# tue-mps/simple-tad

Hardware: AMD Instinct MI355X
Metric: clips/sec (16x224^2 ViT-B) fwd+bwd (higher is better)
Workload: dtype bf16; 1 GPU; vit_base_patch16_224 16x224x224, 32 clips/GPU, fwd+bwd+AdamW fine-tune step with CE loss on synthetic labels (BASELINE configs[2]/[3]); global_batch=32, per_gpu_batch=32, parallelism=dp1, residual_stream=f32, operands=bf16, parameters=86228738

## Files before the change

simple_tad_amd/_lib.py:

```python
from __future__ import annotations

import ctypes as C
import os

_HERE = os.path.dirname(os.path.abspath(__file__))
LIB_PATH = os.environ.get("TAD_LIB") or os.path.join(_HERE, "libtad_mi355x.so")

_vp, _i, _i64, _f, _sz = C.c_void_p, C.c_int, C.c_int64, C.c_float, C.c_size_t

SIGNATURES = {
    "tad_abi_version": (_i, []),
    "tad_last_error_string": (C.c_char_p, []),
    "tad_cast_f32_bf16": (_i, [_vp, _vp, _i64, _vp]),
    "tad_transpose_cast_f32_bf16": (_i, [_vp, _vp, _i, _i, _vp]),
    "tad_patch_embed_ldk": (_i, [_i, _i, _i]),
    "tad_im2col_tubelets": (_i, [_vp, _vp, _i, _i, _i, _i, _i, _i, _i, _vp]),
    "tad_im2col_tubelets_16": (_i, [_vp, _vp, _i, _i, _i, _i, _i, _i, _i, _vp]),
    "tad_patch_embed_fwd": (_i, [_vp, _vp, _vp, _vp, _vp, _vp, _i, _i, _i, _i, _i, _i, _i, _i, _vp]),
    "tad_patch_embed_fwd_implicit": (_i, [_vp, _vp, _vp, _vp, _vp, _i, _i, _i, _i, _i, _i, _i, _i, _vp]),
    "tad_im2col_tubelets_u8": (_i, [_vp, _vp, _i, _i, _i, _i, _i, _i, C.POINTER(_f), C.POINTER(_f), _i, _i, _vp]),
    "tad_im2col_frame_windows": (_i, [_vp, _i64, _vp, _vp, _i, _i, _i, _i, _i, _i, _i, C.POINTER(_f), C.POINTER(_f), _i, _vp]),
    "tad_patch_embed_gemm": (_i, [_vp, _vp, _vp, _vp, _vp, _i64, _i, _i, _i, _vp]),
    "tad_patch_embed_bwd_workspace_bytes": (_sz, [_i64, _i, _i]),
    "tad_patch_embed_bwd": (_i, [_vp, _vp, _vp, _vp, _vp, _sz, _i64, _i, _i, _vp]),
# ... 111 lines not shown
for _bf, _h in (*F16_TWINS.items(), *VARIANT_F16_TWINS.items()):
    SIGNATURES[_h] = SIGNATURES[_bf]
EPI_BIAS, EPI_BIAS_GELU, EPI_BIAS_RESIDUAL = 0, 1, 2
ABI_VERSION = 5

EXT_SIGNATURES = {
    "tadx_abi_version": (_i, []),
    "tadx_rmsnorm_fwd": (_i, [_vp, _vp, _vp, _i, _vp, _i64, _i, _f, _vp]),
    "tadx_rmsnorm_bwd_workspace_bytes": (_sz, [_i64, _i]),
    "tadx_rmsnorm_bwd": (_i, [_vp, _i, _vp, _vp, _vp, _vp, _vp, _vp, _i, _vp, _i, _vp, _sz, _i64, _i, _vp]),
    "tadx_qk_rmsnorm_fwd": (_i, [_vp, _vp, _vp, _vp, _i, _vp, _f, _i64, _i, _f, _vp]),
    "tadx_qk_rmsnorm_bwd_workspace_bytes": (_sz, [_i64, _i]),
    "tadx_qk_rmsnorm_bwd": (_i, [_vp, _i, _vp, _vp, _vp, _vp, _f, _vp, _vp, _vp, _i, _vp, _sz, _i64, _i, _vp]),
}
EXT_ABI_VERSION = 1
LINEAR_PLAN_FIELDS = ("r0", "rows", "kernel", "persistent", "direct", "grid", "block", "group_m", "sk_splits", "sk_mode", "epilogue")
ATTN_PLAN_FIELDS = ("kernel", "hd", "out16", "qs", "drop", "dma_mode", "skip", "has_lo", "grid", "block")
ATTN_FWD, ATTN_FWD_Q64, ATTN_BWD_DQ, ATTN_BWD_DKV = range(4)
LINEAR_BWD_WEIGHT_PLAN_FIELDS = ("N", "tile_k", "tiles", "tiles_k", "splits", "rows_per_split", "kernel", "grid", "block", "pair", "ws_lo", "ws_hi")
ADAMW_CHUNK = 4096
ADAMW_MAX_GROUPS = 128
EMA_CHUNK = 8192
MIXUP_PLAN_WORDS = 12
MIX_KEEP, MIX_BLEND, MIX_PASTE = 0, 1, 2
FRAME_LOSS_KINDS = {"focal": 0, "focal2": 1, "exponential": 2, "2bce": 3, "smoothap": 4}
ERASE_BOX_WORDS = 8
ERASE_CONST, ERASE_RAND, ERASE_PIXEL = 0, 1, 2
RANDAUG_ROW_WORDS = 20
RANDAUG_MAX_LAYERS = 32
(RA_COPY, RA_INVERT, RA_POSTERIZE, RA_SOLARIZE, RA_SOLARIZE_ADD, RA_AUTOCONTRAST, RA_EQUALIZE, RA_BRIGHTNESS, RA_COLOR, RA_CONTRAST,
# ... 12 lines not shown


class TadError(RuntimeError):
    pass


def load() -> C.CDLL:
    global _lib
    if _lib is not None:
        return _lib
    if not os.path.exists(LIB_PATH):
        raise TadError(
            f"{LIB_PATH} not found: the HIP extension has not been built. Run `python -m simple_tad_amd.build` "
            "(or __graft_entry__.build()). There is no CPU fallback for the MI355X path.")
    lib = C.CDLL(LIB_PATH)
    for name, (res, args) in (*SIGNATURES.items(), *EXT_SIGNATURES.items()):
        try:
            fn = getattr(lib, name)
        except AttributeError as e:
            raise TadError(f"{LIB_PATH} does not export {name}") from e
        fn.restype = res
        fn.argtypes = args
    v = lib.tad_abi_version()
    if v != ABI_VERSION:
        raise TadError(f"ABI mismatch: library reports {v}, binding expects {ABI_VERSION}")
    v = lib.tadx_abi_version()
    if v != EXT_ABI_VERSION:
        raise TadError(f"extension ABI mismatch: library reports {v}, binding expects {EXT_ABI_VERSION}")
    _lib = lib
    return lib


def check(rc: int, what: str = "") -> None:
    if rc != 0:
        msg = load().tad_last_error_string()
        raise TadError(f"{what} failed (rc={rc}): {msg.decode() if msg else ''}")
```

simple_tad_amd/build.py:

```python
import os
import subprocess
import sys
from concurrent.futures import ThreadPoolExecutor

HERE = os.path.dirname(os.path.abspath(__file__))
CSRC = os.path.join(HERE, "csrc")
_ABLATION = os.environ.get("TAD_BUILD_ABLATION") == "1"
_LIB_NAME = os.environ.get("TAD_BUILD_LIB", "libtad_ablation.so" if _ABLATION else "libtad_mi355x.so")
EXP_DIR = os.path.join(os.path.dirname(HERE), "build_exp")
_PRODUCTION = _LIB_NAME == "libtad_mi355x.so"
LIB = os.path.join(HERE if _PRODUCTION else EXP_DIR, os.path.basename(_LIB_NAME))
SOURCES = ["capi.hip", "elementwise.hip", "patch_embed.hip", "layernorm.hip", "gemm.hip", "gemm_plan.hip", "gemm_w4.hip", "attn_fwd.hip", "attn_bwd.hip", "attn_plan.hip", "attn_f32.hip", "precise.hip", "optim.hip", "ema.hip", "mixup.hip", "frame_loss.hip", "erasing.hip", "randaug.hip", "multiscale_crop.hip", "frame_resize.hip", "spatial_sample.hip", "mae.hip", "metrics.hip", "group_metrics.hip", "grad_segnorm.hip", "collective.hip", "im2col.hip", "pooled_tail.hip", "layerscale.hip", "attn_colsum.hip", "rmsnorm.hip"]
F16_SOURCES = ["elementwise.hip", "patch_embed.hip", "layernorm.hip", "gemm.hip", "gemm_w4.hip", "attn_fwd.hip", "attn_bwd.hip", "optim.hip", "pooled_tail.hip", "layerscale.hip"]
NO_VGPR_FORM = {"gemm_w4.hip"}
EXTRA_DEPS = {"gemm.hip": ["gemm_kernels.h", "gemm_plan.h"], "gemm_w4.hip": ["gemm_kernels.h", "gemm_plan.h"], "gemm_plan.hip": ["gemm_plan.h", "knob.h"],
              "attn_fwd.hip": ["attn_plan.h"], "attn_bwd.hip": ["attn_plan.h"], "attn_plan.hip": ["attn_plan.h", "knob.h"],
              "multiscale_crop.hip": ["frame_io.h"], "frame_resize.hip": ["frame_io.h"], "spatial_sample.hip": ["frame_io.h"], "randaug.hip": ["frame_io.h"],
              "rmsnorm.hip": ["../../include/tad_mi355x_ext.h"]}
NO_FP_CONTRACT = {"ema.hip", "mixup.hip", "randaug.hip", "multiscale_crop.hip", "spatial_sample.hip", "frame_resize.hip"}
FLAGS = ["--offload-arch=gfx950", "-O3", "-std=c++17", "-fPIC", "-ffp-contract=fast", "-Wno-unused-result",
         "-mllvm", "-amdgpu-mfma-vgpr-form=1"]


def _hipcc():
    for c in (os.environ.get("HIPCC"), "/opt/rocm/bin/hipcc", "hipcc"):
        if c and (os.path.isabs(c) and os.path.exists(c) or not os.path.isabs(c)):
            return c
    return "hipcc"


def _deps_mtime():
    m = 0.0
    for root in (CSRC, os.path.join(os.path.dirname(HERE), "include")):
# ... 46 lines not shown
```

simple_tad_amd/csrc/layernorm.hip:

```cpp
#include "common.h"

TAD_NAMESPACE_BEGIN

constexpr int LN_MAX_V = 8;

int launch_reduce_partials(const float* partial, float* out, int splits, int64_t n, int accumulate, hipStream_t st);
int launch_reduce_cols(const float* partial, float* out0, float* out1, float* out2, int nq, int splits, int n, int accumulate,
                       hipStream_t st);

template <int NV, bool OUT_BF16>
__global__ __launch_bounds__(256) void layernorm_fwd_kernel(const float* __restrict__ x, const float* __restrict__ gamma,
                                                            const float* __restrict__ beta, void* __restrict__ y,
                                                            float* __restrict__ mean, float* __restrict__ rstd,
                                                            int64_t rows, int D, float eps) {
  const int lane = threadIdx.x & 63;
  const int64_t row = (int64_t)blockIdx.x * 4 + (threadIdx.x >> 6);
  if (row >= rows) return;
  const int D4 = D >> 2;
  const float4* xr = reinterpret_cast<const float4*>(x + row * D);
  float4 v[NV];
  float s = 0.f;
#pragma unroll
  for (int i = 0; i < NV; ++i) {
    const int c = lane + 64 * i;
// ... 27 lines not shown
      o.z = (v[i].z - mu) * rs * g.z + b.z;
      o.w = (v[i].w - mu) * rs * g.w + b.w;
      if (OUT_BF16) {
        uint2 p;
        p.x = pack_op16x2(o.x, o.y);
        p.y = pack_op16x2(o.z, o.w);
        stg_u2<false>(reinterpret_cast<uint2*>((uint16_t*)y + row * D) + c, p);
      } else {
        stg_f4<false>(reinterpret_cast<float4*>((float*)y + row * D) + c, o);
      }
    }
  }
}

__device__ const float ln_one = 1.0f;
template <int NV, bool DY_BF16, bool FULL>
__global__ __launch_bounds__(256) void layernorm_bwd_kernel(const void* __restrict__ dy, const float* __restrict__ x,
                                                            const float* __restrict__ gamma, const float* __restrict__ mean,
                                                            const float* __restrict__ rstd, const float* __restrict__ dres,
                                                            float* __restrict__ dx, uint16_t* __restrict__ dxb,
                                                            float* __restrict__ partial , int64_t rows, int D,
                                                            int rows_per_block, int want_colsum,
                                                            const float* __restrict__ rowscale, int rows_per_scale) {
  extern __shared__ __attribute__((aligned(16))) float smem[];
  const int lane = threadIdx.x & 63, wave = __builtin_amdgcn_readfirstlane(threadIdx.x >> 6);
  const int D4 = D >> 2;
  const int64_t r0 = (int64_t)blockIdx.x * rows_per_block;
  const int64_t r1 = min(rows, r0 + rows_per_block);
  float4 g[NV], dg[NV], db[NV], cs[NV];
#pragma unroll
  for (int i = 0; i < NV; ++i) {
    const int c = lane + 64 * i;
    g[i] = (c < D4) ? reinterpret_cast<const float4*>(gamma)[c] : make_float4(0.f, 0.f, 0.f, 0.f);
    dg[i] = db[i] = cs[i] = make_float4(0.f, 0.f, 0.f, 0.f);
  }
  const float* const rsrc = dres ? dres : x;
  const float rmul = dres ? 1.f : 0.f;
  const float* const scp = rowscale ? rowscale : &ln_one;
  int sidx = 0, srem = 0;
  if (rowscale) {
    sidx = (int)((r0 + wave) / rows_per_scale);
    srem = (int)((r0 + wave) - (int64_t)sidx * rows_per_scale);
  }
  for (int64_t row = r0 + wave; row < r1; row += 4) {
    float4 xv[NV], dyv[NV], rv[NV];
    uint2 dyp[NV];
#pragma unroll
    for (int i = 0; i < NV; ++i) {
      const int c = lane + 64 * i;
      if (FULL || c < D4) {
        xv[i] = ldg_f4<false>(reinterpret_cast<const float4*>(x + row * D) + c);
        if (DY_BF16) dyp[i] = ldg_u2<false>(reinterpret_cast<const uint2*>((const uint16_t*)dy + row * D) + c);
        else dyv[i] = ldg_f4<false>(reinterpret_cast<const float4*>((const float*)dy + row * D) + c);
        rv[i] = ldg_f4<false>(reinterpret_cast<const float4*>(rsrc + row * D) + c);
      }
    }
    const float mu = mean[row], rs = rstd[row];
    const float sc = scp[sidx];
    if (rowscale) {
      srem += 4;
      while (srem >= rows_per_scale) { srem -= rows_per_scale; ++sidx; }
    }
    __builtin_amdgcn_sched_barrier(0);
    float4 xh[NV];
    float s1 = 0.f, s2 = 0.f;
#pragma unroll
    for (int i = 0; i < NV; ++i) {
      const int c = lane + 64 * i;
      if (FULL || c < D4) {
        if (DY_BF16)
          dyv[i] = make_float4(op16_lo_f32(dyp[i].x), op16_hi_f32(dyp[i].x), op16_lo_f32(dyp[i].y), op16_hi_f32(dyp[i].y));
        xh[i] = make_float4((xv[i].x - mu) * rs, (xv[i].y - mu) * rs, (xv[i].z - mu) * rs, (xv[i].w - mu) * rs);
        const float4 t = make_float4(dyv[i].x * g[i].x, dyv[i].y * g[i].y, dyv[i].z * g[i].z, dyv[i].w * g[i].w);
        s1 += (t.x + t.y) + (t.z + t.w);
        s2 += (t.x * xh[i].x + t.y * xh[i].y) + (t.z * xh[i].z + t.w * xh[i].w);
        dg[i].x += dyv[i].x * xh[i].x; dg[i].y += dyv[i].y * xh[i].y; dg[i].z += dyv[i].z * xh[i].z; dg[i].w += dyv[i].w * xh[i].w;
// ... 51 lines not shown
    for (int w = 1; w < 4; ++w) {
      const float4 b = sm[(w * 3 + q) * D4 + c];
      a.x += b.x; a.y += b.y; a.z += b.z; a.w += b.w;
    }
    reinterpret_cast<float4*>(partial + ((int64_t)q * gridDim.x + blockIdx.x) * D)[c] = a;
  }
}

static inline int ln_bwd_blocks(int64_t rows) {
  int64_t b = (rows + 31) / 32;
  if (b > 1024) b = 1024;
  if (b < 1) b = 1;
  return (int)b;
}

TAD_NAMESPACE_END

using namespace tad;

extern "C" {

int tad_layernorm_fwd(const float* x, const float* gamma, const float* beta, void* y, int y_dtype, float* mean, float* rstd,
                      int64_t rows, int D, float eps, tad_stream_t stream) {
  TAD_REQUIRE(x && gamma && beta && y, "layernorm_fwd: null pointer");
  TAD_REQUIRE(rows > 0 && D > 0 && D % 4 == 0 && D <= 64 * 4 * LN_MAX_V, "layernorm_fwd: D=%d must be a multiple of 4 and <= %d", D,
              64 * 4 * LN_MAX_V);
  TAD_REQUIRE(y_dtype == TAD_F32 || y_dtype == TAD_OP16, "layernorm_fwd: bad y_dtype %d", y_dtype);
  TAD_REQUIRE_ALIGNED("layernorm_fwd", x, 16);
  TAD_REQUIRE_ALIGNED("layernorm_fwd", gamma, 16);
  TAD_REQUIRE_ALIGNED("layernorm_fwd", beta, 16);
  TAD_REQUIRE_ALIGNED("layernorm_fwd", y, y_dtype == TAD_F32 ? 16 : 8);
// ... 14 lines not shown
    case 6: LN_FWD(6); break;
    default: LN_FWD(8); break;
  }
#undef LN_FWD
  return check_launch("layernorm_fwd");
}

#ifndef TAD_OPND_F16
size_t tad_layernorm_bwd_workspace_bytes(int64_t rows, int D) { return (size_t)3 * ln_bwd_blocks(rows) * (size_t)D * sizeof(float); }
#endif

int tad_layernorm_bwd(const void* dy, int dy_dtype, const float* x, const float* gamma, const float* mean, const float* rstd,
                      const float* dres, float* dx, uint16_t* dx_bf16, float* dgamma, float* dbeta, float* colsum_dx,
                      const float* rowscale, int rows_per_scale, int accumulate, void* ws, size_t ws_bytes, int64_t rows, int D,
                      tad_stream_t stream) {
  TAD_REQUIRE(dy && x && gamma && mean && rstd && dx && dgamma && dbeta && ws, "layernorm_bwd: null pointer");
  TAD_REQUIRE(rows > 0 && D > 0 && D % 4 == 0 && D <= 64 * 4 * LN_MAX_V, "layernorm_bwd: unsupported D=%d", D);
  TAD_REQUIRE(dy_dtype == TAD_F32 || dy_dtype == TAD_OP16, "layernorm_bwd: bad dy_dtype %d", dy_dtype);
  TAD_REQUIRE(!rowscale || rows_per_scale > 0, "layernorm_bwd: rows_per_scale must be positive");
  TAD_REQUIRE_ALIGNED("layernorm_bwd", dy, dy_dtype == TAD_F32 ? 16 : 8);
  TAD_REQUIRE_ALIGNED("layernorm_bwd", x, 16);
  TAD_REQUIRE_ALIGNED("layernorm_bwd", gamma, 16);
  TAD_REQUIRE_ALIGNED("layernorm_bwd", dres, 16);
  TAD_REQUIRE_ALIGNED("layernorm_bwd", dx, 16);
  TAD_REQUIRE_ALIGNED("layernorm_bwd", dx_bf16, 8);
  TAD_REQUIRE_ALIGNED("layernorm_bwd", dgamma, 16);
  TAD_REQUIRE_ALIGNED("layernorm_bwd", dbeta, 16);
  TAD_REQUIRE_ALIGNED("layernorm_bwd", colsum_dx, 16);
  TAD_REQUIRE_ALIGNED("layernorm_bwd", ws, 16);
  const int blocks = ln_bwd_blocks(rows);
  if (ws_bytes < (size_t)3 * blocks * D * sizeof(float)) { set_error("layernorm_bwd: workspace too small"); return TAD_ENOSPACE; }
  const int rows_per_block = (int)((rows + blocks - 1) / blocks);
  const int nv = (D / 4 + 63) / 64;
  const size_t smem = (size_t)4 * 3 * D * sizeof(float);
  hipStream_t st = (hipStream_t)stream;
  float* partial = (float*)ws;
  const int want_cs = colsum_dx != nullptr;
  const bool full = (D == 256 * nv);
#define LN_BWD_(NV, BF, FULL_)                                                                                                  \
  hipLaunchKernelGGL((layernorm_bwd_kernel<NV, BF, FULL_>), dim3(blocks), dim3(256), smem, st, dy, x, gamma, mean, rstd, dres, dx, \
                     dx_bf16, partial, rows, D, rows_per_block, want_cs, rowscale, rows_per_scale)
#define LN_BWD(NV)                                                                                                             \
  if (dy_dtype == TAD_OP16) { if (full) LN_BWD_(NV, true, true); else LN_BWD_(NV, true, false); }                               \
  else { if (full) LN_BWD_(NV, false, true); else LN_BWD_(NV, false, false); }
  switch (nv) {
    case 1: LN_BWD(1); break;
    case 2: LN_BWD(2); break;
    case 3: LN_BWD(3); break;
    case 4: LN_BWD(4); break;
    case 5: LN_BWD(5); break;
    case 6: LN_BWD(6); break;
    default: LN_BWD(8); break;
  }
#undef LN_BWD
#undef LN_BWD_
  int rc = check_launch("layernorm_bwd");
  if (rc) return rc;
  rc = launch_reduce_cols(partial, dgamma, dbeta, colsum_dx, colsum_dx ? 3 : 2, blocks, D, accumulate ? 1 : 0, st);
  return rc;
}

}
```

simple_tad_amd/kernels.py:

```python
from __future__ import annotations

import ctypes as C
from typing import Optional

import torch

from . import _lib
from ._lib import EPI_BIAS, EPI_BIAS_GELU, EPI_BIAS_RESIDUAL, TAD_BF16, TAD_F16, TAD_F32, check

_workspaces = {}


class LaunchProfiler:

    def __init__(self, only=None, stride=1):
        self.items = []
        self.only = set(only) if only else None
        self.stride = max(1, int(stride))
        self.seen = {}

    def wants(self, kernel):
        if self.only is not None and kernel not in self.only:
            return False
        n = self.seen.get(kernel, 0)
# ... 419 lines not shown
    _req(x, torch.float32, "layernorm.x")
    _req(gamma, torch.float32, "layernorm.gamma")
    _req(beta, torch.float32, "layernorm.beta")
    D = x.shape[-1]
    rows = x.numel() // D
    y = torch.empty(x.shape, dtype=out_dtype or _op16, device=x.device)
    mean = torch.empty(rows, dtype=torch.float32, device=x.device) if save_stats else None
    rstd = torch.empty(rows, dtype=torch.float32, device=x.device) if save_stats else None
    with _timed("layernorm_fwd", 0.0, rows * D * (4.0 + y.element_size())):
        check(_fn("tad_layernorm_fwd", y.dtype if y.dtype in OP16_DTYPES else _op16)(x.data_ptr(), gamma.data_ptr(), beta.data_ptr(), y.data_ptr(), _dt(y), _p(mean), _p(rstd),
                                            rows, D, float(eps), _stream()), "tad_layernorm_fwd")
    return y, mean, rstd


def layernorm_bwd(dy, x, gamma, mean, rstd, dres=None, want_bf16=False, want_colsum=False, rowscale=None, rows_per_scale=1,
                  into=None):
    _req(x, torch.float32, "layernorm_bwd.x")
    if dy.dtype not in (torch.float32,) + OP16_DTYPES or not dy.is_contiguous():
        raise _lib.TadError("layernorm_bwd.dy: must be contiguous f32, bf16 or f16")
    op = dy.dtype if dy.dtype in OP16_DTYPES else _op16
    D = x.shape[-1]
    rows = x.numel() // D
    if dres is not None:
        _req(dres, torch.float32, "layernorm_bwd.dres")
    dx = torch.empty(x.shape, dtype=torch.float32, device=x.device)
    dxb = torch.empty(x.shape, dtype=op, device=x.device) if want_bf16 else None
    if into is not None:
        dg, db, cs = into
        for t in (dg, db) + ((cs,) if want_colsum else ()):
            _req(t, torch.float32, "layernorm_bwd.into")
            assert t.numel() == D
        if not want_colsum:
            cs = None
    else:
        dg = torch.empty(D, dtype=torch.float32, device=x.device)
        db = torch.empty(D, dtype=torch.float32, device=x.device)
        cs = torch.empty(D, dtype=torch.float32, device=x.device) if want_colsum else None
    if rowscale is not None:
        _req(rowscale, torch.float32, "layernorm_bwd.rowscale")
        assert rowscale.numel() * rows_per_scale >= rows
    lib = _lib.load()
    nbytes = lib.tad_layernorm_bwd_workspace_bytes(rows, D)
    ws = workspace(nbytes, x.device)
    with _timed("layernorm_bwd", 0.0, rows * D * (dy.element_size() + 4.0 + 4.0 + (4.0 if dres is not None else 0.0) + (2.0 if want_bf16 else 0.0))):
        check(_fn("tad_layernorm_bwd", op)(dy.data_ptr(), _dt(dy), x.data_ptr(), gamma.data_ptr(), mean.data_ptr(), rstd.data_ptr(), _p(dres),
                                    dx.data_ptr(), _p(dxb), dg.data_ptr(), db.data_ptr(), _p(cs), _p(rowscale), int(rows_per_scale),
                                    int(into is not None), ws.data_ptr(), ws.numel(), rows, D, _stream()), "tad_layernorm_bwd")
    return dx, dxb, dg, db, cs


def _ext(name: str):
    return getattr(_lib.load(), name)


def rmsnorm_fwd(x, gamma, eps: float, out_dtype=None, save_stats=True):
    _req(x, torch.float32, "rmsnorm.x")
    _req(gamma, torch.float32, "rmsnorm.gamma")
    D = x.shape[-1]
# ... 1054 lines not shown
```

simple_tad_amd/ops.py:

```python
from __future__ import annotations

import contextlib
import threading
import weakref
from typing import Optional

import torch

from . import kernels as K
from ._lib import EPI_BIAS, EPI_BIAS_GELU, EPI_BIAS_RESIDUAL, TadError

_wcache = {}
_static = {}
_MAKERS = {}


def invalidate_weight_cache(keep_static: bool = False):
    global _weight_epoch
    _weight_epoch += 1
    _wcache.clear()
    if not keep_static:
        _static.clear()
    _mirrors.clear()
    _mirrors_t.clear()
# ... 261 lines not shown
    @staticmethod
    def backward(ctx, dy):
        xc, w, mean, rstd = ctx.saved_tensors
        D = xc.shape[-1]
        dx, _, dg, db, _ = K.layernorm_bwd(_f32c(dy).reshape(-1, D), xc.reshape(-1, D), w, mean, rstd)
        return dx.reshape(xc.shape), dg, db, None


IMPLICIT_PATCH_EMBED_MIN_TILES = 512


def _patch_embed_backward(ctx, dy, trailing: int):
    weight, bias = ctx.params
    need_w, need_b = ctx.need
    need_b = need_b and bias is not None
    if not (need_w or need_b):
        return (None, None) + (None,) * trailing
    dyb = K.cast_bf16(_f32c(dy).reshape(-1, dy.shape[-1]))
    if not need_w:
        return (None, K.colsum_bf16(dyb)) + (None,) * trailing
    (cols,) = ctx.saved_tensors
    if not need_b:
        bias = None
    kw = weight.numel() // weight.shape[0]
    if cols.shape[1] != kw:
        dWp, db = K.linear_bwd_weight(dyb, cols, want_bias=bias is not None)
        dW = dWp[:, :kw]
    else:
        dW, db = linear_dw(dyb, cols, weight, bias)
    return (None if dW is None else dW.reshape(weight.shape), db) + (None,) * trailing


class PatchEmbedFn(_Fn):

    @staticmethod
    def forward(ctx, x, weight, bias, pos, tubelet, patch):
        _need_gpu(x, "PatchEmbed")
        xc = _f32c(x)
        ldk = K.patch_embed_ldk(xc.shape[1], tubelet, patch)
        ntok_ = (xc.shape[2] // tubelet) * (xc.shape[3] // patch) * (xc.shape[4] // patch)
        ctx.need = _needs(ctx, 3)[1:]
        keeps_cols = _differentiated(ctx) and ctx.need[0]
        if not keeps_cols and -(-xc.shape[0] * ntok_ // 128) * -(-weight.shape[0] // 128) >= IMPLICIT_PATCH_EMBED_MIN_TILES:
            out = K.patch_embed_fwd_implicit(xc, w_bf16(weight, _differentiated(ctx)), _f32c(bias), _f32c(pos), tubelet, patch)
            if out is not None:
                ctx.params = (weight, bias)
                return out
        out, cols = K.patch_embed_fwd(xc, K.pad_k(w_bf16(weight, _differentiated(ctx)), ldk), _f32c(bias), _f32c(pos), tubelet, patch)
        if ctx.need[0]:
            ctx.save_for_backward(cols)
        ctx.params = (weight, bias)
        return out

    @staticmethod
    def backward(ctx, dy):
        return (None,) + _patch_embed_backward(ctx, dy, 3)


class PatchEmbed16Fn(_Fn):

    @staticmethod
    def forward(ctx, x, weight, bias, pos, tubelet, patch):
        _need_gpu(x, "PatchEmbed")
        xc = x.detach()
        xc = xc if xc.is_contiguous() else xc.contiguous()
        cols = K.im2col_tubelets_16(xc, tubelet, patch)
        if cols is None:
            cols = K.im2col_tubelets(xc.float(), tubelet, patch, dtype=xc.dtype)
        ntok = (xc.shape[2] // tubelet) * (xc.shape[3] // patch) * (xc.shape[4] // patch)
        out = K.patch_embed_gemm(cols, K.pad_k(w_bf16(weight, _differentiated(ctx)), cols.shape[1]), _f32c(bias), _f32c(pos), ntok)
        ctx.need = _needs(ctx, 3)[1:]
        if ctx.need[0]:
            ctx.save_for_backward(cols)
        ctx.params = (weight, bias)
        return out

    @staticmethod
    def backward(ctx, dy):
        return (None,) + _patch_embed_backward(ctx, dy, 3)


class PatchEmbedU8Fn(_Fn):

    @staticmethod
    def forward(ctx, frames, weight, bias, pos, tubelet, patch, mean, std, bgr, t_offset):
        _need_gpu(frames, "PatchEmbed")
        fr = frames if frames.is_contiguous() else frames.contiguous()
        B, T, H, W, _ = fr.shape
        cols = K.im2col_tubelets_u8(fr, tubelet, patch, mean, std, bgr, t_offset)
        ntok = (T // tubelet) * (H // patch) * (W // patch)
        out = K.patch_embed_gemm(cols, K.pad_k(w_bf16(weight, _differentiated(ctx)), cols.shape[1]), _f32c(bias), _f32c(pos), ntok)
        ctx.need = _needs(ctx, 3)[1:]
        if ctx.need[0]:
            ctx.save_for_backward(cols)
        ctx.params = (weight, bias)
        return out

    @staticmethod
    def backward(ctx, dy):
        return (None,) + _patch_embed_backward(ctx, dy, 7)


class PatchEmbedWindowsFn(_Fn):

    @staticmethod
    def forward(ctx, store, idx, weight, bias, pos, tubelet, patch, mean, std, bgr):
        _need_gpu(store, "PatchEmbed")
        B, T = idx.shape
        _, H, W, _ = store.shape
        cols = K.im2col_frame_windows(store, idx, tubelet, patch, mean, std, bgr)
        ntok = (T // tubelet) * (H // patch) * (W // patch)
        out = K.patch_embed_gemm(cols, K.pad_k(w_bf16(weight, _differentiated(ctx)), cols.shape[1]), _f32c(bias), _f32c(pos), ntok)
        ctx.need = _needs(ctx, 4)[2:]
        if ctx.need[0]:
            ctx.save_for_backward(cols)
        ctx.params = (weight, bias)
        return out

# ... 355 lines not shown
        return dx, dWqkv, dbqkv, dgq, dgk, dWp, dbp, None, None, None


class _ChainLink:
    __slots__ = ("dp2", "deposit", "__weakref__")

    def __init__(self, dp2):
        self.dp2 = dp2
        self.deposit = None


class _ChainState:
    def __init__(self):
        self.enabled = True
        self.hits = 0
        self.pending = 0


_chain = _ChainState()


def reset_block_chain():
    """kept for API compatibility: the hand-off state lives in per-forward link objects and needs no reset"""


def set_block_chain(enabled: bool):
    _chain.enabled = bool(enabled)


def block_apply(x, *args):
# ... 57 lines not shown
    a, h = K.linear_fwd(xn2, w_bf16(fc1_w, train), _f32c(fc1_b), out_dtype=None, epilogue=EPI_BIAS_GELU, want_preact=train)
    need = ctx.need = _needs(ctx, 14)
    if train:
        ctx.save_for_backward(x0, g1, mean1, rstd1, xn1 if need[3] else None, qkv, ao, lse, x1, g2, mean2, rstd2, xn2 if need[10] else None,
                              h, a if need[12] else None, qkv_w, proj_w, fc1_w, fc2_w,
                              dp1 if dp1 is None else _f32c(dp1), dp2 if dp2 is None else _f32c(dp2), ao_lo)
    ctx.meta = (B, N, D, H, scale, q_bias is not None)
    ctx.biases = (proj_b, fc1_b, fc2_b)
    ctx.norms = (n1w, n1b, n2w, n2b)
    ctx.qv = (q_bias, v_bias)
    ctx.prev_link = prev_link if train else None
    ctx.link = link if train else None
    return train, x1, a


def _block_bwd_from_dh(ctx, st, g, dh, dW2, db2):
    x0, g1, mean1, rstd1, xn1, qkv, ao, lse, x1, g2, mean2, rstd2, xn2, h, a, qkv_w, proj_w, fc1_w, fc2_w, dp1, dp2, ao_lo = st
    proj_b, fc1_b, fc2_b = ctx.biases
    B, N, D, H, scale, has_qb = ctx.meta
    dxn2 = K.linear_bwd_input(dh, wT_bf16(fc1_w, True))
    need = ctx.need
    dW1, db1 = linear_dw(dh, xn2, fc1_w, fc1_b, need=need[10:12])
    n1w, n1b, n2w, n2b = ctx.norms
    gmid, gpb, dg2, dbeta2, dbp = layernorm_bwd_sunk(dxn2, x1, g2, mean2, rstd2, n2w, n2b, colsum_param=proj_b if need[7] else None, dres=g,
                                                    want_bf16=True, rowscale=dp1, rows_per_scale=N)
    d_ao = K.linear_bwd_input(gpb, wT_bf16(proj_w, True))
    dxn1, dWqkv, dqb, dvb, dWp = _attn_bwd_core(d_ao, xn1, qkv, ao, lse, qkv_w, has_qb, B, N, H, scale, None, ctx.qv, ao_lo=ao_lo, q_prescaled=ctx.qpre,
                                                 pair=(gpb, ao, proj_w), rowscale=dp1, need=need[3:6], pair_need=need[6])
    prev = ctx.prev_link
    if prev is not None:
        gin, ginb, dg1, dbeta1, _ = layernorm_bwd_sunk(dxn1, x0, g1, mean1, rstd1, n1w, n1b, dres=gmid, want_bf16=True, rowscale=prev.dp2,
                                                       rows_per_scale=N)
        if prev.deposit is None:
            _chain.pending += 1
        prev.deposit = (ginb, gin, gin._version)
    else:
        gin, _, dg1, dbeta1, _ = layernorm_bwd_sunk(dxn1, x0, g1, mean1, rstd1, n1w, n1b, dres=gmid)
    return (gin.reshape(B, N, D), dg1, dbeta1, dWqkv, dqb, dvb, dWp, dbp, dg2, dbeta2, dW1, db1, dW2, db2, None, None, None, None,
            None, None, None)

# ... 105 lines not shown
        dxn2 = K.linear_bwd_input(dh, wT_bf16(fc1_w, True))
        dW1, db1 = linear_dw(dh, xn2, fc1_w, fc1_b, need=need[10:12])
        gmid, gpb, dg2, dbeta2, _ = layernorm_bwd_sunk(dxn2, x1, g2, mean2, rstd2, n2w, n2b, dres=g, want_bf16=p == 0.0, rowscale=dp1,
                                                     rows_per_scale=N)
        if p > 0.0:
            gpb = K.branch_dropout_cast(gmid, dp1, N, p, seed_attn)
        d_ao = K.linear_bwd_input(gpb, _branch_wT(proj_w, gm1))
        dWp, dbp, dgm1 = _branch_dw(gpb, ao, proj_w, proj_b, gamma_1, gm1, need=(need[6], need[7], need[14]))
        dxn1, dWqkv, dqb, dvb = _attn_bwd_core(d_ao, xn1, qkv, ao, lse, qkv_w, has_qb, B, N, H, scale, None, ctx.qv, ao_lo=ao_lo,
                                               q_prescaled=ctx.qpre, rowscale=dp1, need=need[3:6])
        gin, _, dg1, dbeta1, _ = layernorm_bwd_sunk(dxn1, x0, g1, mean1, rstd1, n1w, n1b, dres=gmid)
        return (gin.reshape(B, N, D), dg1, dbeta1, dWqkv, dqb, dvb, dWp, dbp, dg2, dbeta2, dW1, db1, dW2, db2, dgm1, dgm2, None, None,
                None, None, None, None, None, None)


_pooled_tail = None


def set_pooled_tail(enabled: bool):
    global _pooled_tail
    _pooled_tail = bool(enabled)


def get_pooled_tail() -> bool:
    global _pooled_tail
    if _pooled_tail is None:
        import os
        v = os.environ.get("TAD_POOLED_TAIL", "1").strip()
        _pooled_tail = not (v.isdigit() and int(v) == 0)
    return _pooled_tail


def pooled_tail_ok(fc2_w) -> bool:
    return get_pooled_tail() and _PRECISION in ("fast", "half") and K.colsum_segments_ok(fc2_w.shape[1])


class _PoolStats:
    calls = 0


def block_pool_apply(x, *args):
    prev = getattr(x, "_tad_link", None) if _chain.enabled else None
    _PoolStats.calls += 1
    return BlockPoolFn.apply(x, *args, prev, None)


class BlockPoolFn(_Fn):

    @staticmethod
    def forward(ctx, x, n1w, n1b, qkv_w, q_bias, v_bias, proj_w, proj_b, n2w, n2b, fc1_w, fc1_b, fc2_w, fc2_b, dp1, dp2, H, scale,
                eps, prev_link=None, link=None):
        train, x1, a = _block_fwd_to_fc1(ctx, x, n1w, n1b, qkv_w, q_bias, v_bias, proj_w, proj_b, n2w, n2b, fc1_w, fc1_b, fc2_w, fc2_b,
                                         dp1, dp2, H, scale, eps, prev_link, link)
        B, N, D = x.shape
        S = K.colsum_segments(a, B, N)
        xbar = K.meanpool_fwd(x1.view(B, N, D))
        ctx.pool_S = S if train and ctx.need[12] else None
        return K.pooled_linear(S, w_bf16(fc2_w, train), _f32c(fc2_b), _f32c(dp2), xbar, N)

    @staticmethod
    def backward(ctx, dy):
        st = ctx.saved_tensors
        h, fc2_w, dp2 = st[13], st[18], st[20]
        S = ctx.pool_S
        B, N, D = ctx.meta[:3]
        fc2_b = ctx.biases[2]
        g, _ = K.meanpool_bwd(_f32c(dy), N)
        g_rows = g[:, 0, :].contiguous()
        gb = K.cast_bf16(g_rows) if dp2 is None else K.scale_cast_bf16(g_rows, None, dp2, 1)
        t = K.linear_bwd_input(gb, wT_bf16(fc2_w, True), out_dtype=torch.float32)
        dh = K.gelu_grad_bcast(t, h, N)
        need_w, need_b = ctx.need[12], ctx.need[13] and fc2_b is not None
        if not need_w:
            return _block_bwd_from_dh(ctx, st, g.view(B * N, D), dh, None, gb.float().sum(0) * float(N) if need_b else None)
        if not need_b:
            fc2_b = None
        gbf = gb.float()
        sw = _sink(fc2_w)
        sb = _sink(fc2_b) if fc2_b is not None else None
        if sw is not None and (fc2_b is None or sb is not None):
            sw[1].view(fc2_w.shape[0], -1).addmm_(gbf.t(), S)
            if sb is not None:
                sb[1].add_(gbf.sum(0), alpha=float(N))
            for ent, prm in ((sw, fc2_w), (sb, fc2_b)):
                if ent is not None and ent[2] is not None:
                    ent[2](prm)
            dW2, db2 = None, None
        else:
            dW2 = torch.matmul(gbf.t(), S)
            db2 = gbf.sum(0) * float(N) if fc2_b is not None else None
        return _block_bwd_from_dh(ctx, st, g.view(B * N, D), dh, dW2, db2)


class LinearFn(_Fn):

    @staticmethod
    def forward(ctx, x, weight, bias):
        _need_gpu(x, "Linear")
        shp = x.shape
        train = _differentiated(ctx)
        ctx.params = (weight, bias)
        ctx.shp = shp
        ctx.precise = _PRECISION == "precise"
        if ctx.precise:
            x2 = _f32c(x).reshape(-1, shp[-1])
            y = precise_linear(x2, weight, bias, fresh=train)
# ... 188 lines not shown
```

Baseline: 734.2 clips/sec.

## Broadcast pooled residual gradient in LayerNorm backward and chain patch-embed bf16 cast

In the pooled-tail last block, the mean-pool backward no longer expands dy into a full B*N*D residual gradient. LayerNorm backward gets a broadcast variant that reads one residual-gradient row per N token rows, exposed through a new extension entry point with an ABI check. Patch-embed backward can now reuse a bf16 copy of dy deposited by the chained block, skipping a separate cast. This cuts memory traffic and a materialization at both ends of the encoder, at the cost of more template instantiations and extra version-checking logic.

```diff
diff --git a/include/tad_mi355x_ext2.h b/include/tad_mi355x_ext2.h
--- /dev/null
+++ b/include/tad_mi355x_ext2.h
@@ -0,0 +1,23 @@
+#ifndef TAD_MI355X_EXT2_H
+#define TAD_MI355X_EXT2_H
+
+#include "tad_mi355x.h"
+
+#ifdef __cplusplus
+extern "C" {
+#endif
+
+#define TADX2_ABI_VERSION 1
+
+int tadx2_abi_version(void);
+
+int tadx2_layernorm_bwd_bcast(const void* dy, int dy_dtype, const float* x, const float* gamma, const float* mean, const float* rstd,
+                              const float* dres, int rows_per_dres, float* dx, uint16_t* dx_bf16, int fmt, float* dgamma, float* dbeta,
+                              float* colsum_dx, const float* rowscale, int rows_per_scale, int accumulate, void* ws, size_t ws_bytes,
+                              int64_t rows, int D, tad_stream_t stream);
+
+#ifdef __cplusplus
+}
+#endif
+
+#endif
diff --git a/simple_tad_amd/_lib.py b/simple_tad_amd/_lib.py
--- a/simple_tad_amd/_lib.py
+++ b/simple_tad_amd/_lib.py
@@ -149,6 +149,11 @@
     "tadx_qk_rmsnorm_bwd": (_i, [_vp, _i, _vp, _vp, _vp, _vp, _f, _vp, _vp, _vp, _i, _vp, _sz, _i64, _i, _vp]),
 }
 EXT_ABI_VERSION = 1
+EXT2_SIGNATURES = {
+    "tadx2_abi_version": (_i, []),
+    "tadx2_layernorm_bwd_bcast": (_i, [_vp, _i, _vp, _vp, _vp, _vp, _vp, _i, _vp, _vp, _i, _vp, _vp, _vp, _vp, _i, _i, _vp, _sz, _i64, _i, _vp]),
+}
+EXT2_ABI_VERSION = 1
 LINEAR_PLAN_FIELDS = ("r0", "rows", "kernel", "persistent", "direct", "grid", "block", "group_m", "sk_splits", "sk_mode", "epilogue")
 ATTN_PLAN_FIELDS = ("kernel", "hd", "out16", "qs", "drop", "dma_mode", "skip", "has_lo", "grid", "block")
 ATTN_FWD, ATTN_FWD_Q64, ATTN_BWD_DQ, ATTN_BWD_DKV = range(4)
@@ -191,7 +196,7 @@
             f"{LIB_PATH} not found: the HIP extension has not been built. Run `python -m simple_tad_amd.build` "
             "(or __graft_entry__.build()). There is no CPU fallback for the MI355X path.")
     lib = C.CDLL(LIB_PATH)
-    for name, (res, args) in (*SIGNATURES.items(), *EXT_SIGNATURES.items()):
+    for name, (res, args) in (*SIGNATURES.items(), *EXT_SIGNATURES.items(), *EXT2_SIGNATURES.items()):
         try:
             fn = getattr(lib, name)
         except AttributeError as e:
@@ -204,6 +209,9 @@
     v = lib.tadx_abi_version()
     if v != EXT_ABI_VERSION:
         raise TadError(f"extension ABI mismatch: library reports {v}, binding expects {EXT_ABI_VERSION}")
+    v = lib.tadx2_abi_version()
+    if v != EXT2_ABI_VERSION:
+        raise TadError(f"second extension ABI mismatch: library reports {v}, binding expects {EXT2_ABI_VERSION}")
     _lib = lib
     return lib
 
diff --git a/simple_tad_amd/build.py b/simple_tad_amd/build.py
--- a/simple_tad_amd/build.py
+++ b/simple_tad_amd/build.py
@@ -16,7 +16,7 @@
 EXTRA_DEPS = {"gemm.hip": ["gemm_kernels.h", "gemm_plan.h"], "gemm_w4.hip": ["gemm_kernels.h", "gemm_plan.h"], "gemm_plan.hip": ["gemm_plan.h", "knob.h"],
               "attn_fwd.hip": ["attn_plan.h"], "attn_bwd.hip": ["attn_plan.h"], "attn_plan.hip": ["attn_plan.h", "knob.h"],
               "multiscale_crop.hip": ["frame_io.h"], "frame_resize.hip": ["frame_io.h"], "spatial_sample.hip": ["frame_io.h"], "randaug.hip": ["frame_io.h"],
-              "rmsnorm.hip": ["../../include/tad_mi355x_ext.h"]}
+              "rmsnorm.hip": ["../../include/tad_mi355x_ext.h"], "layernorm.hip": ["../../include/tad_mi355x_ext2.h"]}
 NO_FP_CONTRACT = {"ema.hip", "mixup.hip", "randaug.hip", "multiscale_crop.hip", "spatial_sample.hip", "frame_resize.hip"}
 FLAGS = ["--offload-arch=gfx950", "-O3", "-std=c++17", "-fPIC", "-ffp-contract=fast", "-Wno-unused-result",
          "-mllvm", "-amdgpu-mfma-vgpr-form=1"]
diff --git a/simple_tad_amd/csrc/layernorm.hip b/simple_tad_amd/csrc/layernorm.hip
--- a/simple_tad_amd/csrc/layernorm.hip
+++ b/simple_tad_amd/csrc/layernorm.hip
@@ -65,14 +65,15 @@
 }
 
 __device__ const float ln_one = 1.0f;
-template <int NV, bool DY_BF16, bool FULL>
+template <int NV, bool DY_BF16, bool FULL, bool BCAST = false>
 __global__ __launch_bounds__(256) void layernorm_bwd_kernel(const void* __restrict__ dy, const float* __restrict__ x,
                                                             const float* __restrict__ gamma, const float* __restrict__ mean,
                                                             const float* __restrict__ rstd, const float* __restrict__ dres,
                                                             float* __restrict__ dx, uint16_t* __restrict__ dxb,
                                                             float* __restrict__ partial , int64_t rows, int D,
                                                             int rows_per_block, int want_colsum,
-                                                            const float* __restrict__ rowscale, int rows_per_scale) {
+                                                            const float* __restrict__ rowscale, int rows_per_scale,
+                                                            int rows_per_dres) {
   extern __shared__ __attribute__((aligned(16))) float smem[];
   const int lane = threadIdx.x & 63, wave = __builtin_amdgcn_readfirstlane(threadIdx.x >> 6);
   const int D4 = D >> 2;
@@ -93,8 +94,14 @@
     sidx = (int)((r0 + wave) / rows_per_scale);
     srem = (int)((r0 + wave) - (int64_t)sidx * rows_per_scale);
   }
+  int didx = 0, drem = 0;
+  if (BCAST) {
+    didx = (int)((r0 + wave) / rows_per_dres);
+    drem = (int)((r0 + wave) - (int64_t)didx * rows_per_dres);
+  }
   for (int64_t row = r0 + wave; row < r1; row += 4) {
     float4 xv[NV], dyv[NV], rv[NV];
+    const int64_t rrow = BCAST ? (int64_t)didx : row;
     uint2 dyp[NV];
 #pragma unroll
     for (int i = 0; i < NV; ++i) {
@@ -103,7 +110,7 @@
         xv[i] = ldg_f4<false>(reinterpret_cast<const float4*>(x + row * D) + c);
         if (DY_BF16) dyp[i] = ldg_u2<false>(reinterpret_cast<const uint2*>((const uint16_t*)dy + row * D) + c);
         else dyv[i] = ldg_f4<false>(reinterpret_cast<const float4*>((const float*)dy + row * D) + c);
-        rv[i] = ldg_f4<false>(reinterpret_cast<const float4*>(rsrc + row * D) + c);
+        rv[i] = ldg_f4<false>(reinterpret_cast<const float4*>(rsrc + rrow * D) + c);
       }
     }
     const float mu = mean[row], rs = rstd[row];
@@ -111,6 +118,10 @@
     if (rowscale) {
       srem += 4;
       while (srem >= rows_per_scale) { srem -= rows_per_scale; ++sidx; }
+    }
+    if (BCAST) {
+      drem += 4;
+      while (drem >= rows_per_dres) { drem -= rows_per_dres; ++didx; }
     }
     __builtin_amdgcn_sched_barrier(0);
     float4 xh[NV];
@@ -192,7 +203,71 @@
   return (int)b;
 }
 
+int ln_bwd_launch(const char* who, const void* dy, int dy_dtype, const float* x, const float* gamma, const float* mean, const float* rstd,
+                  const float* dres, int rows_per_dres, float* dx, uint16_t* dx_bf16, float* dgamma, float* dbeta, float* colsum_dx,
+                  const float* rowscale, int rows_per_scale, int accumulate, void* ws, size_t ws_bytes, int64_t rows, int D,
+                  tad_stream_t stream) {
+  TAD_REQUIRE(dy && x && gamma && mean && rstd && dx && dgamma && dbeta && ws, "%s: null pointer", who);
+  TAD_REQUIRE(rows > 0 && D > 0 && D % 4 == 0 && D <= 64 * 4 * LN_MAX_V, "%s: unsupported D=%d", who, D);
+  TAD_REQUIRE(dy_dtype == TAD_F32 || dy_dtype == TAD_OP16, "%s: bad dy_dtype %d", who, dy_dtype);
+  TAD_REQUIRE(!rowscale || rows_per_scale > 0, "%s: rows_per_scale must be positive", who);
+  TAD_REQUIRE_ALIGNED(who, dy, dy_dtype == TAD_F32 ? 16 : 8);
+  TAD_REQUIRE_ALIGNED(who, x, 16);
+  TAD_REQUIRE_ALIGNED(who, gamma, 16);
+  TAD_REQUIRE_ALIGNED(who, dres, 16);
+  TAD_REQUIRE_ALIGNED(who, dx, 16);
+  TAD_REQUIRE_ALIGNED(who, dx_bf16, 8);
+  TAD_REQUIRE_ALIGNED(who, dgamma, 16);
+  TAD_REQUIRE_ALIGNED(who, dbeta, 16);
+  TAD_REQUIRE_ALIGNED(who, colsum_dx, 16);
+  TAD_REQUIRE_ALIGNED(who, ws, 16);
+  const int blocks = ln_bwd_blocks(rows);
+  if (ws_bytes < (size_t)3 * blocks * D * sizeof(float)) { set_error("%s: workspace too small", who); return TAD_ENOSPACE; }
+  const int rows_per_block = (int)((rows + blocks - 1) / blocks);
+  const int nv = (D / 4 + 63) / 64;
+  const size_t smem = (size_t)4 * 3 * D * sizeof(float);
+  hipStream_t st = (hipStream_t)stream;
+  float* partial = (float*)ws;
+  const int want_cs = colsum_dx != nullptr;
+  const bool full = (D == 256 * nv);
+  const bool bcast = rows_per_dres > 0;
+#define LN_BWD__(NV, BF, FULL_, BC)                                                                                                     \
+  hipLaunchKernelGGL((layernorm_bwd_kernel<NV, BF, FULL_, BC>), dim3(blocks), dim3(256), smem, st, dy, x, gamma, mean, rstd, dres, dx, \
+                     dx_bf16, partial, rows, D, rows_per_block, want_cs, rowscale, rows_per_scale, rows_per_dres)
+#define LN_BWD_(NV, BF, FULL_) \
+  if (bcast) LN_BWD__(NV, BF, FULL_, true); else LN_BWD__(NV, BF, FULL_, false)
+#define LN_BWD(NV)                                                                                  \
+  if (dy_dtype == TAD_OP16) { if (full) { LN_BWD_(NV, true, true); } else { LN_BWD_(NV, true, false); } } \
+  else { if (full) { LN_BWD_(NV, false, true); } else { LN_BWD_(NV, false, false); } }
+  switch (nv) {
+    case 1: LN_BWD(1); break;
+    case 2: LN_BWD(2); break;
+    case 3: LN_BWD(3); break;
+    case 4: LN_BWD(4); break;
+    case 5: LN_BWD(5); break;
+    case 6: LN_BWD(6); break;
+    default: LN_BWD(8); break;
+  }
+#undef LN_BWD
+#undef LN_BWD_
+#undef LN_BWD__
+  int rc = check_launch(who);
+  if (rc) return rc;
+  rc = launch_reduce_cols(partial, dgamma, dbeta, colsum_dx, colsum_dx ? 3 : 2, blocks, D, accumulate ? 1 : 0, st);
+  return rc;
+}
+
 TAD_NAMESPACE_END
+
+#ifndef TAD_OPND_F16
+namespace tad { namespace op_f16 {
+int ln_bwd_launch(const char* who, const void* dy, int dy_dtype, const float* x, const float* gamma, const float* mean, const float* rstd,
+                  const float* dres, int rows_per_dres, float* dx, uint16_t* dx_bf16, float* dgamma, float* dbeta, float* colsum_dx,
+                  const float* rowscale, int rows_per_scale, int accumulate, void* ws, size_t ws_bytes, int64_t rows, int D,
+                  tad_stream_t stream);
+}}
+#include "../../include/tad_mi355x_ext2.h"
+#endif
 
 using namespace tad;
 
@@ -237,50 +312,26 @@
                       const float* dres, float* dx, uint16_t* dx_bf16, float* dgamma, float* dbeta, float* colsum_dx,
                       const float* rowscale, int rows_per_scale, int accumulate, void* ws, size_t ws_bytes, int64_t rows, int D,
                       tad_stream_t stream) {
-  TAD_REQUIRE(dy && x && gamma && mean && rstd && dx && dgamma && dbeta && ws, "layernorm_bwd: null pointer");
-  TAD_REQUIRE(rows > 0 && D > 0 && D % 4 == 0 && D <= 64 * 4 * LN_MAX_V, "layernorm_bwd: unsupported D=%d", D);
-  TAD_REQUIRE(dy_dtype == TAD_F32 || dy_dtype == TAD_OP16, "layernorm_bwd: bad dy_dtype %d", dy_dtype);
-  TAD_REQUIRE(!rowscale || rows_per_scale > 0, "layernorm_bwd: rows_per_scale must be positive");
-  TAD_REQUIRE_ALIGNED("layernorm_bwd", dy, dy_dtype == TAD_F32 ? 16 : 8);
-  TAD_REQUIRE_ALIGNED("layernorm_bwd", x, 16);
-  TAD_REQUIRE_ALIGNED("layernorm_bwd", gamma, 16);
-  TAD_REQUIRE_ALIGNED("layernorm_bwd", dres, 16);
-  TAD_REQUIRE_ALIGNED("layernorm_bwd", dx, 16);
-  TAD_REQUIRE_ALIGNED("layernorm_bwd", dx_bf16, 8);
-  TAD_REQUIRE_ALIGNED("layernorm_bwd", dgamma, 16);
-  TAD_REQUIRE_ALIGNED("layernorm_bwd", dbeta, 16);
-  TAD_REQUIRE_ALIGNED("layernorm_bwd", colsum_dx, 16);
-  TAD_REQUIRE_ALIGNED("layernorm_bwd", ws, 16);
-  const int blocks = ln_bwd_blocks(rows);
-  if (ws_bytes < (size_t)3 * blocks * D * sizeof(float)) { set_error("layernorm_bwd: workspace too small"); return TAD_ENOSPACE; }
-  const int rows_per_block = (int)((rows + blocks - 1) / blocks);
-  const int nv = (D / 4 + 63) / 64;
-  const size_t smem = (size_t)4 * 3 * D * sizeof(float);
-  hipStream_t st = (hipStream_t)stream;
-  float* partial = (float*)ws;
-  const int want_cs = colsum_dx != nullptr;
-  const bool full = (D == 256 * nv);
-#define LN_BWD_(NV, BF, FULL_)                                                                                                  \
-  hipLaunchKernelGGL((layernorm_bwd_kernel<NV, BF, FULL_>), dim3(blocks), dim3(256), smem, st, dy, x, gamma, mean, rstd, dres, dx, \
-                     dx_bf16, partial, rows, D, rows_per_block, want_cs, rowscale, rows_per_scale)
-#define LN_BWD(NV)                                                                                                             \
-  if (dy_dtype == TAD_OP16) { if (full) LN_BWD_(NV, true, true); else LN_BWD_(NV, true, false); }                               \
-  else { if (full) LN_BWD_(NV, false, true); else LN_BWD_(NV, false, false); }
-  switch (nv) {
-    case 1: LN_BWD(1); break;
-    case 2: LN_BWD(2); break;
-    case 3: LN_BWD(3); break;
-    case 4: LN_BWD(4); break;
-    case 5: LN_BWD(5); break;
-    case 6: LN_BWD(6); break;
-    default: LN_BWD(8); break;
-  }
-#undef LN_BWD
-#undef LN_BWD_
-  int rc = check_launch("layernorm_bwd");
-  if (rc) return rc;
-  rc = launch_reduce_cols(partial, dgamma, dbeta, colsum_dx, colsum_dx ? 3 : 2, blocks, D, accumulate ? 1 : 0, st);
-  return rc;
-}
-
-}
+  return ln_bwd_launch("layernorm_bwd", dy, dy_dtype, x, gamma, mean, rstd, dres, 0, dx, dx_bf16, dgamma, dbeta, colsum_dx, rowscale,
+                       rows_per_scale, accumulate, ws, ws_bytes, rows, D, stream);
+}
+
+#ifndef TAD_OPND_F16
+int tadx2_abi_version(void) { return TADX2_ABI_VERSION; }
+
+int tadx2_layernorm_bwd_bcast(const void* dy, int dy_dtype, const float* x, const float* gamma, const float* mean, const float* rstd,
+                              const float* dres, int rows_per_dres, float* dx, uint16_t* dx_bf16, int fmt, float* dgamma, float* dbeta,
+                              float* colsum_dx, const float* rowscale, int rows_per_scale, int accumulate, void* ws, size_t ws_bytes,
+                              int64_t rows, int D, tad_stream_t stream) {
+  static const char who[] = "layernorm_bwd_bcast";
+  TAD_REQUIRE(fmt == TAD_BF16 || fmt == TAD_F16, "%s: bad fmt %d", who, fmt);
+  TAD_REQUIRE(dy_dtype == TAD_F32 || dy_dtype == fmt, "%s: bad dy_dtype %d (f32, or the call's 16-bit format %d)", who, dy_dtype, fmt);
+  TAD_REQUIRE(dres, "%s: null pointer", who);
+  TAD_REQUIRE(rows_per_dres > 0, "%s: rows_per_dres must be positive", who);
+  return (fmt == TAD_F16 ? op_f16::ln_bwd_launch : op_bf16::ln_bwd_launch)(who, dy, dy_dtype, x, gamma, mean, rstd, dres, rows_per_dres, dx,
+                                                                          dx_bf16, dgamma, dbeta, colsum_dx, rowscale, rows_per_scale,
+                                                                          accumulate, ws, ws_bytes, rows, D, stream);
+}
+#endif
+
+}
diff --git a/simple_tad_amd/kernels.py b/simple_tad_amd/kernels.py
--- a/simple_tad_amd/kernels.py
+++ b/simple_tad_amd/kernels.py
@@ -457,7 +457,7 @@
 
 
 def layernorm_bwd(dy, x, gamma, mean, rstd, dres=None, want_bf16=False, want_colsum=False, rowscale=None, rows_per_scale=1,
-                  into=None):
+                  into=None, rows_per_dres=0):
     _req(x, torch.float32, "layernorm_bwd.x")
     if dy.dtype not in (torch.float32,) + OP16_DTYPES or not dy.is_contiguous():
         raise _lib.TadError("layernorm_bwd.dy: must be contiguous f32, bf16 or f16")
@@ -466,6 +466,9 @@
     rows = x.numel() // D
     if dres is not None:
         _req(dres, torch.float32, "layernorm_bwd.dres")
+    if rows_per_dres:
+        if dres is None or rows_per_dres < 0 or dres.numel() != -(-rows // rows_per_dres) * D:
+            raise _lib.TadError(f"layernorm_bwd.dres: rows_per_dres={rows_per_dres} needs a residual gradient of {-(-rows // max(rows_per_dres, 1))} rows")
     dx = torch.empty(x.shape, dtype=torch.float32, device=x.device)
     dxb = torch.empty(x.shape, dtype=op, device=x.device) if want_bf16 else None
     if into is not None:
@@ -485,6 +488,13 @@
     lib = _lib.load()
     nbytes = lib.tad_layernorm_bwd_workspace_bytes(rows, D)
     ws = workspace(nbytes, x.device)
+    if rows_per_dres:
+        with _timed("layernorm_bwd", 0.0, rows * D * (dy.element_size() + 4.0 + 4.0 + (2.0 if want_bf16 else 0.0))):
+            check(lib.tadx2_layernorm_bwd_bcast(dy.data_ptr(), _dt(dy), x.data_ptr(), gamma.data_ptr(), mean.data_ptr(), rstd.data_ptr(),
+                                                dres.data_ptr(), int(rows_per_dres), dx.data_ptr(), _p(dxb), TAD_F16 if op == torch.float16 else TAD_BF16,
+                                                dg.data_ptr(), db.data_ptr(), _p(cs), _p(rowscale), int(rows_per_scale), int(into is not None),
+                                                ws.data_ptr(), ws.numel(), rows, D, _stream()), "tadx2_layernorm_bwd_bcast")
+        return dx, dxb, dg, db, cs
     with _timed("layernorm_bwd", 0.0, rows * D * (dy.element_size() + 4.0 + 4.0 + (4.0 if dres is not None else 0.0) + (2.0 if want_bf16 else 0.0))):
         check(_fn("tad_layernorm_bwd", op)(dy.data_ptr(), _dt(dy), x.data_ptr(), gamma.data_ptr(), mean.data_ptr(), rstd.data_ptr(), _p(dres),
                                     dx.data_ptr(), _p(dxb), dg.data_ptr(), db.data_ptr(), _p(cs), _p(rowscale), int(rows_per_scale),
diff --git a/simple_tad_amd/ops.py b/simple_tad_amd/ops.py
--- a/simple_tad_amd/ops.py
+++ b/simple_tad_amd/ops.py
@@ -299,9 +299,21 @@
     weight, bias = ctx.params
     need_w, need_b = ctx.need
     need_b = need_b and bias is not None
+    dy2 = _f32c(dy).reshape(-1, dy.shape[-1])
+    dyb = None
+    link = getattr(ctx, "link", None)
+    dep = link.deposit if link is not None else None
+    if dep is not None:
+        link.deposit = None
+        _chain.pending -= 1
+        cand, ref, ver = dep
+        if ref.data_ptr() == dy2.data_ptr() and ref._version == ver and dy2._version == ver and cand.shape == dy2.shape:
+            dyb = cand
+            _chain.embed_hits += 1
     if not (need_w or need_b):
         return (None, None) + (None,) * trailing
-    dyb = K.cast_bf16(_f32c(dy).reshape(-1, dy.shape[-1]))
+    if dyb is None:
+        dyb = K.cast_bf16(dy2)
     if not need_w:
         return (None, K.colsum_bf16(dyb)) + (None,) * trailing
     (cols,) = ctx.saved_tensors
@@ -316,7 +328,19 @@
     return (None if dW is None else dW.reshape(weight.shape), db) + (None,) * trailing
 
 
-class PatchEmbedFn(_Fn):
+class _PatchEmbedFn(_Fn):
+
+    @classmethod
+    def apply(cls, *args, **kwargs):
+        out = super().apply(*args, **kwargs)
+        if _chain.enabled and get_encoder_ends() and torch.is_grad_enabled() and out.requires_grad:
+            node = out.grad_fn
+            if getattr(node, "params", None) is not None:
+                node.link = out._tad_link = _ChainLink(None)
+        return out
+
+
+class PatchEmbedFn(_PatchEmbedFn):
 
     @staticmethod
     def forward(ctx, x, weight, bias, pos, tubelet, patch):
@@ -342,7 +366,7 @@
         return (None,) + _patch_embed_backward(ctx, dy, 3)
 
 
-class PatchEmbed16Fn(_Fn):
+class PatchEmbed16Fn(_PatchEmbedFn):
 
     @staticmethod
     def forward(ctx, x, weight, bias, pos, tubelet, patch):
@@ -365,7 +389,7 @@
         return (None,) + _patch_embed_backward(ctx, dy, 3)
 
 
-class PatchEmbedU8Fn(_Fn):
+class PatchEmbedU8Fn(_PatchEmbedFn):
 
     @staticmethod
     def forward(ctx, frames, weight, bias, pos, tubelet, patch, mean, std, bgr, t_offset):
@@ -386,7 +410,7 @@
         return (None,) + _patch_embed_backward(ctx, dy, 7)
 
 
-class PatchEmbedWindowsFn(_Fn):
+class PatchEmbedWindowsFn(_PatchEmbedFn):
 
     @staticmethod
     def forward(ctx, store, idx, weight, bias, pos, tubelet, patch, mean, std, bgr):
@@ -772,6 +796,7 @@
     def __init__(self):
         self.enabled = True
         self.hits = 0
+        self.embed_hits = 0
         self.pending = 0
 
 
@@ -859,7 +884,7 @@
     return train, x1, a
 
 
-def _block_bwd_from_dh(ctx, st, g, dh, dW2, db2):
+def _block_bwd_from_dh(ctx, st, g, dh, dW2, db2, rows_per_g=0):
     x0, g1, mean1, rstd1, xn1, qkv, ao, lse, x1, g2, mean2, rstd2, xn2, h, a, qkv_w, proj_w, fc1_w, fc2_w, dp1, dp2, ao_lo = st
     proj_b, fc1_b, fc2_b = ctx.biases
     B, N, D, H, scale, has_qb = ctx.meta
@@ -868,7 +893,7 @@
     dW1, db1 = linear_dw(dh, xn2, fc1_w, fc1_b, need=need[10:12])
     n1w, n1b, n2w, n2b = ctx.norms
     gmid, gpb, dg2, dbeta2, dbp = layernorm_bwd_sunk(dxn2, x1, g2, mean2, rstd2, n2w, n2b, colsum_param=proj_b if need[7] else None, dres=g,
-                                                    want_bf16=True, rowscale=dp1, rows_per_scale=N)
+                                                    want_bf16=True, rowscale=dp1, rows_per_scale=N, rows_per_dres=rows_per_g)
     d_ao = K.linear_bwd_input(gpb, wT_bf16(proj_w, True))
     dxn1, dWqkv, dqb, dvb, dWp = _attn_bwd_core(d_ao, xn1, qkv, ao, lse, qkv_w, has_qb, B, N, H, scale, None, ctx.qv, ao_lo=ao_lo, q_prescaled=ctx.qpre,
                                                  pair=(gpb, ao, proj_w), rowscale=dp1, need=need[3:6], pair_need=need[6])
@@ -1004,6 +1029,23 @@
                 None, None, None, None, None, None)
 
 
+_encoder_ends = None
+
+
+def set_encoder_ends(enabled: bool):
+    global _encoder_ends
+    _encoder_ends = bool(enabled)
+
+
+def get_encoder_ends() -> bool:
+    global _encoder_ends
+    if _encoder_ends is None:
+        import os
+        v = os.environ.get("TAD_ENCODER_ENDS", "1").strip()
+        _encoder_ends = not (v.isdigit() and int(v) == 0)
+    return _encoder_ends
+
+
 _pooled_tail = None
 
 
@@ -1033,6 +1075,10 @@
     prev = getattr(x, "_tad_link", None) if _chain.enabled else None
     _PoolStats.calls += 1
     return BlockPoolFn.apply(x, *args, prev, None)
+
+
+def _inv_f32(n: int) -> float:
+    return float(torch.tensor(1.0, dtype=torch.float32) / torch.tensor(float(n), dtype=torch.float32))
 
 
 class BlockPoolFn(_Fn):
@@ -1046,6 +1092,7 @@
         S = K.colsum_segments(a, B, N)
         xbar = K.meanpool_fwd(x1.view(B, N, D))
         ctx.pool_S = S if train and ctx.need[12] else None
+        ctx.ends = get_encoder_ends()
         return K.pooled_linear(S, w_bf16(fc2_w, train), _f32c(fc2_b), _f32c(dp2), xbar, N)
 
     @staticmethod
@@ -1055,14 +1102,19 @@
         S = ctx.pool_S
         B, N, D = ctx.meta[:3]
         fc2_b = ctx.biases[2]
-        g, _ = K.meanpool_bwd(_f32c(dy), N)
-        g_rows = g[:, 0, :].contiguous()
+        if ctx.ends:
+            g_rows = _f32c(dy) * _inv_f32(N)
+            g, bc = g_rows, N
+        else:
+            g3, _ = K.meanpool_bwd(_f32c(dy), N)
+            g_rows = g3[:, 0, :].contiguous()
+            g, bc = g3.view(B * N, D), 0
         gb = K.cast_bf16(g_rows) if dp2 is None else K.scale_cast_bf16(g_rows, None, dp2, 1)
         t = K.linear_bwd_input(gb, wT_bf16(fc2_w, True), out_dtype=torch.float32)
         dh = K.gelu_grad_bcast(t, h, N)
         need_w, need_b = ctx.need[12], ctx.need[13] and fc2_b is not None
         if not need_w:
-            return _block_bwd_from_dh(ctx, st, g.view(B * N, D), dh, None, gb.float().sum(0) * float(N) if need_b else None)
+            return _block_bwd_from_dh(ctx, st, g, dh, None, gb.float().sum(0) * float(N) if need_b else None, rows_per_g=bc)
         if not need_b:
             fc2_b = None
         gbf = gb.float()
@@ -1079,7 +1131,7 @@
         else:
             dW2 = torch.matmul(gbf.t(), S)
             db2 = gbf.sum(0) * float(N) if fc2_b is not None else None
-        return _block_bwd_from_dh(ctx, st, g.view(B * N, D), dh, dW2, db2)
+        return _block_bwd_from_dh(ctx, st, g, dh, dW2, db2, rows_per_g=bc)
 
 
 class LinearFn(_Fn):
```

New measurement: 734.8 clips/sec (median of 2 runs). No clear change (+0.1%).
